# emuell/AFEC

Measured on AMD Instinct MI355X. Metric: audio frames/sec low-level crawl, 44.1kHz 1024-hop, higher is better.
Workload: dtype f64

## Files before the change

### afec_amd/csrc/afx_frames32.hip

```cpp

#include <hip/hip_runtime.h>

#include "afx_internal.h"
#include "afx_device.h"
#include "afx_fft32.h"

namespace afx {
namespace {

using f32x32::cx;

constexpr int kHalfSlots = 1056;
constexpr int kPlane32Bytes = 2 * kHalfSlots * 8;
constexpr int kWaves32 = 8;

template <int POST_ROWS>
struct Lds32 {
  static constexpr int tw = 0;
  static constexpr int post = tw + 32 * 32 * 16;
  static constexpr int dct = post + POST_ROWS * 32 * 16;
  static constexpr int logc = dct + 14 * 16 * 8;
  static constexpr int xchg = logc + 32 * 8;
  static constexpr int total = xchg + kWaves32 * kPlane32Bytes;
};

__device__ __forceinline__ __amdgpu_buffer_rsrc_t table_rsrc(const void* p, int bytes) {
  return __builtin_amdgcn_make_buffer_rsrc(const_cast<void*>(p), 0, bytes, 0x00020000);
}
typedef unsigned int u32x4_t __attribute__((ext_vector_type(4)));
typedef unsigned int u32x2_t __attribute__((ext_vector_type(2)));
__device__ __forceinline__ double2 table_load2(__amdgpu_buffer_rsrc_t rs, int lane_off, int row_off) {
  return __builtin_bit_cast(double2, __builtin_amdgcn_raw_buffer_load_b128(rs, lane_off, row_off, 0));
}
__device__ __forceinline__ double table_load1(__amdgpu_buffer_rsrc_t rs, int lane_off, int row_off) {
  return __builtin_bit_cast(double, __builtin_amdgcn_raw_buffer_load_b64(rs, lane_off, row_off, 0));
}

template <int IMM, bool NT>
__device__ __forceinline__ void dma_piece(const void* gaddr, unsigned lds_base) {
  if constexpr (NT)
    asm volatile("s_mov_b32 m0, %1\n\ts_nop 0\n\tglobal_load_lds_dwordx4 %0, off offset:%2 nt"
                 :: "v"(gaddr), "s"(lds_base), "n"(IMM) : "memory", "m0");
  else
    asm volatile("s_mov_b32 m0, %1\n\ts_nop 0\n\tglobal_load_lds_dwordx4 %0, off offset:%2"
                 :: "v"(gaddr), "s"(lds_base), "n"(IMM) : "memory", "m0");
}
template <bool NT = true>
__device__ __forceinline__ void dma_hop(const float* g, unsigned lds_plane) {
  dma_piece<0, NT>(g, lds_plane);
  dma_piece<512, NT>(g, lds_plane + 512);
  dma_piece<1024, NT>(g, lds_plane + 1024);
  dma_piece<1536, NT>(g, lds_plane + 1536);
  dma_piece<2048, NT>(g, lds_plane + 2048);
  dma_piece<2560, NT>(g, lds_plane + 2560);
  dma_piece<3072, NT>(g, lds_plane + 3072);
  dma_piece<3584, NT>(g, lds_plane + 3584);
}

__device__ __forceinline__ double mag_sqrt_mel(double xr, double xi, double tiny, double three) {
  const double x = fma(xi, xi, fma(xr, xr, tiny));
  const double r = __builtin_amdgcn_rsq(x);
  const double y = x * r;
  return y * fma(-r, y, three);
}

__device__ __forceinline__ void keep_lane0(double& re, double& im, double own_re, double own_im, unsigned long long lane0_mask) {
  unsigned long long saved;
  asm volatile("s_mov_b64 %2, exec\n\ts_mov_b64 exec, %5\n\tv_mov_b64 %0, %3\n\tv_mov_b64 %1, %4\n\ts_mov_b64 exec, %2"
               : "+v"(re), "+v"(im), "=&s"(saved) : "v"(own_re), "v"(own_im), "s"(lane0_mask));
}

__device__ __forceinline__ double half_sum16(double (&a)[16], int lane) {
#pragma unroll
  for (int i = 0; i < 8; ++i) {
    swap16(a[i], a[i + 8]);
    a[i] += a[i + 8];
  }
  const bool b3 = (lane & 8) != 0, b2 = (lane & 4) != 0, b1 = (lane & 2) != 0;
#pragma unroll
  for (int i = 0; i < 4; ++i) {
    const double keep = b3 ? a[i + 4] : a[i];
    const double send = b3 ? a[i] : a[i + 4];
    a[i] = keep + dpp_mov<kDppRor8>(send);
  }
#pragma unroll
  for (int i = 0; i < 2; ++i) {
    const double keep = b2 ? a[i + 2] : a[i];
    const double send = b2 ? a[i] : a[i + 2];
    a[i] = keep + dpp_mov<kDppHalfMirror>(send);
  }
  const double keep = b1 ? a[1] : a[0];
  const double send = b1 ? a[0] : a[1];
  double z = keep + dpp_mov<kDppXor2>(send);
  z += dpp_mov<kDppXor1>(z);
  return z;
}

__device__ const double kLogConst[32] = {1.0 / 23.0, 1.0 / 21.0, 1.0 / 19.0, 1.0 / 17.0, 1.0 / 15.0, 1.0 / 13.0,
                                         1.0 / 11.0, 1.0 / 9.0,  1.0 / 7.0,  1.0 / 5.0,  1.0 / 3.0,  0.693147180559945309417,
                                         0.70710678118654752440, 2e-42,
                                         1e-20, 32.0, 0.38268343236508984, -0.9238795325112867, 1.0 / 738.0,
                                         (double)(85.0f / 100.0), 43.0, -1.0 / 60.0, (double)1e-12f, 3.0,
                                         1.44269504088896340736, 20.0 / 2.30258509299404568402, 2.2250738585072014e-308, 3.33547137486383e-154 , 511.0, 0.0, 0.0, 0.0};
constexpr int kCEps = 14, kC32 = 15, kCRotRe = 16, kCRotIm = 17, kCRoll = 19, kCSqrtMin = 27, kC511 = 28;

__device__ __forceinline__ double log_lds(double x, const double* c) {
  double m = __builtin_amdgcn_frexp_mant(x);
  int e = __builtin_amdgcn_frexp_exp(x);
  const bool lowhalf = m < c[12];
// ... 4 lines not shown
  double p = c[0];
#pragma unroll
  for (int i = 1; i < 11; ++i) p = fma(p, z, c[i]);
  p = fma(p, z, 1.0);
  return fma((double)e, c[11], 2.0 * s * p);
}

__device__ __forceinline__ void finish_mfcc32(double acc, double*& recp, int& left, int stride2, const double* dct,
                                              const double* logc, int lane) {
  const double lg = log_lds(fmax(acc, logc[13]), logc);
  int ln = lane;
  asm volatile("" : "+v"(ln));
  const int n = (ln >> 1) & 15;
  const double2* drow = reinterpret_cast<const double2*>(dct + 16 * (n < kNumCep ? n : 0));
  const int idx = ((ln & 32) + (ln & 1)) << 2;
  const int lo32 = __double2loint(lg), hi32 = __double2hiint(lg);
  double c = 0.0;
#pragma unroll
  for (int m = 0; m < kNumCep; m += 2) {
    const double2 d = drow[m >> 1];
    const double l0 = __hiloint2double(__builtin_amdgcn_ds_bpermute(idx + 8 * m, hi32), __builtin_amdgcn_ds_bpermute(idx + 8 * m, lo32));
    const double l1 = __hiloint2double(__builtin_amdgcn_ds_bpermute(idx + 8 * m + 8, hi32), __builtin_amdgcn_ds_bpermute(idx + 8 * m + 8, lo32));
    c = fma(l0, d.x, c);
    c = fma(l1, d.y, c);
  }
  if (n < kNumCep && left > 0) *recp = c;
  recp += stride2;
  left -= 2;
}

#ifndef AFX_STAMPS
#define AFX_STAMPS 0
#endif
#if AFX_STAMPS
#define AFX_STAMP(i)                                                                           \
  do {                                                                                         \
    unsigned long long t_;                                                                     \
    asm volatile("s_memtime %0\n\ts_waitcnt lgkmcnt(0)" : "=s"(t_));                           \
    stamp_acc[i] += (unsigned)(t_ - stamp_prev);                                               \
    stamp_prev = t_;                                                                           \
  } while (0)
#else
#define AFX_STAMP(i)
#endif


template <int FEAT, bool SCALED>
__global__ __launch_bounds__(kWaves32 * 64) void frames32_kernel(const FrameArgs a) {
  constexpr bool MAGS = (FEAT == 4 || FEAT == 6);
  constexpr bool MAGS_UPPER = (FEAT == 4);
  constexpr int kMelEarly = 4;
  constexpr bool LO_LDS = (FEAT >= 2 && FEAT <= 4) || FEAT == 6;
  constexpr bool kHopNt = !LO_LDS;
  constexpr bool kLoNt = true;
  constexpr bool STATS = (FEAT >= 1 && FEAT <= 3) || FEAT == 5;
  constexpr bool MOMENTS34 = (FEAT != 5);
  constexpr bool PAIRS = STATS;
  constexpr bool STORE = (FEAT == 2 || FEAT == 3);
  constexpr bool UPPER = (FEAT == 3);
  constexpr int MR = (FEAT >= 1) ? 16 : kMel32Rows;
  using Map = Lds32<kMel32Rows>;
  extern __shared__ __align__(16) unsigned char lds_raw[];
  const int lane = threadIdx.x & 63;
  const int wave = __builtin_amdgcn_readfirstlane(threadIdx.x >> 6);
  const int h = lane >> 5, q = lane & 31;

  copy_lds_table(lds_raw + Map::tw, a.tw32, 32 * 32 * 16, threadIdx.x, kWaves32 * 64);
  copy_lds_table(lds_raw + Map::post, a.post32, kMel32Rows * 32 * 16, threadIdx.x, kWaves32 * 64);
  copy_lds_table(lds_raw + Map::dct, a.dct, 14 * 16 * 8, threadIdx.x, kWaves32 * 64);
  copy_lds_table(lds_raw + Map::logc, kLogConst, 32 * 8, threadIdx.x, kWaves32 * 64);
#if AFX_STAMPS
  unsigned stamp_acc[16] = {};
  unsigned long long life_core0, life_real0;
  asm volatile("s_memtime %0\n\ts_memrealtime %1\n\ts_waitcnt lgkmcnt(0)" : "=s"(life_core0), "=s"(life_real0));
  const bool stamping = (wave == 0) && a.stamps != nullptr;
  unsigned long long stamp_prev = 0;
#endif
  __syncthreads();

  const __amdgpu_buffer_rsrc_t win_rs = table_rsrc(a.win32, 32 * 32 * 16);
  const __amdgpu_buffer_rsrc_t mel_rs = table_rsrc(a.melw32, kMel32Pairs * 32 * 8);
  const int q16 = 16 * q, q8 = 8 * q;
  const double2* const tw = reinterpret_cast<const double2*>(lds_raw + Map::tw) + q;
  const double2* const post = reinterpret_cast<const double2*>(lds_raw + Map::post) + q;
  const double* const dct = reinterpret_cast<const double*>(lds_raw + Map::dct);
  const double* const logc = reinterpret_cast<const double*>(lds_raw + Map::logc);
  const int stride2 = 2 * a.lay.stride;
  double* const plane = reinterpret_cast<double*>(lds_raw + Map::xchg + wave * kPlane32Bytes) + kHalfSlots * h;
  double* const pw = plane + q;
  using lds_vdouble = volatile __attribute__((address_space(3))) double;
  lds_vdouble* const pr = (lds_vdouble*)(plane + 33 * q);
  const int partner = (lane & 32) + ((32 - q) & 31);
  const int dh = (lane >> 4) & 1, drow = lane >> 5, dq = 2 * (lane & 15);
  typedef __attribute__((address_space(3))) void lvoid;
  unsigned char* const plane_bytes = lds_raw + Map::xchg + wave * kPlane32Bytes;
  const unsigned plane_lds = __builtin_amdgcn_readfirstlane((unsigned)(size_t)(lvoid*)plane_bytes);
  double k_tiny = 2.2250738585072014e-308, k_three = 3.0;
  unsigned long long k_lane0 = 0x0000000100000001ull;
  asm volatile("" : "+s"(k_tiny), "+s"(k_three), "+s"(k_lane0));
  lds_vdouble* const hop = (lds_vdouble*)(plane_bytes + 256 * h + 8 * q);

  const float* const pcm = reinterpret_cast<const float*>(a.pcm);

  const int n_items = (a.n_chunks + 1) >> 1;
  const int n_static = min((int)(gridDim.x * kWaves32), n_items);
  for (int slot = blockIdx.x * kWaves32 + wave; slot < n_items;) {
    const int ci = 2 * slot + h;
    const bool have = ci < a.n_chunks;
    const Chunk ch = a.chunks[have ? ci : 2 * slot];
    const int nfr = have ? ch.nframes : 0;
    const double sc = ch.scale;
    const int total = max(__builtin_amdgcn_readlane(nfr, 0), __builtin_amdgcn_readlane(nfr, 32));
    const float2* src = reinterpret_cast<const float2*>(pcm + ch.sample_off) + q;
    const int cid = 2 * slot + dh;
    const bool have_d = cid < a.n_chunks;
    const Chunk chd = a.chunks[have_d ? cid : 2 * slot];
    const int last_d = max((have_d ? (int)chd.nframes : 0) - 1, 0);
    const float* const dsrc = pcm + chd.sample_off + 64 * (16 + drow) + 2 * dq;

    double lo[16];
    if constexpr (!LO_LDS) {
      const double* const src8 = reinterpret_cast<const double*>(src);
#pragma unroll
      for (int r = 0; r < 16; ++r) lo[r] = src8[32 * r];
    } else {
      dma_hop<kLoNt>(dsrc - kHop, plane_lds + 8192);
    }
    dma_hop<kHopNt>(dsrc, plane_lds);

    double mel_acc = 0.0;
    double* recp = a.rec + ((int64_t)ch.frame0 + (q & 1)) * a.lay.stride + a.lay.mfcc + ((q >> 1) & 15);
    int left = nfr - (q & 1);

    double2 w[32];
#pragma unroll
    for (int r = 0; r < 32; ++r) w[r] = table_load2(win_rs, q16, 512 * r);

#if AFX_STAMPS
    asm volatile("s_memtime %0\n\ts_waitcnt lgkmcnt(0)" : "=s"(stamp_prev));
#endif
    for (int fi = 0; fi < total; ++fi) {
      cx<double> v[32];
      {
        double nx[16];
        asm volatile("s_waitcnt vmcnt(0)" ::: "memory");
        AFX_STAMP(0);
#pragma unroll
        for (int r = 0; r < 16; ++r) nx[r] = hop[64 * r];
        __builtin_amdgcn_sched_barrier(0);
        if constexpr (LO_LDS) {
          const double* const lo_rows = reinterpret_cast<const double*>(plane_bytes + 8192 + 256 * h) + q;
#pragma unroll
          for (int r = 0; r < 16; ++r) lo[r] = lo_rows[64 * r];
        }
        double hop_sq = 0.0, hop_max = 0.0;
#pragma unroll
        for (int j = 0; j < 8; ++j) {
          auto first = [](double pair) { return __int_as_float(__double2loint(pair)); };
          auto second = [](double pair) { return __int_as_float(__double2hiint(pair)); };
          const double ar = pcm_double<SCALED>(first(lo[j]), sc), ai = pcm_double<SCALED>(second(lo[j]), sc);
          const double br = pcm_double<SCALED>(first(lo[j + 8]), sc), bi = pcm_double<SCALED>(second(lo[j + 8]), sc);
          const double cr = pcm_double<SCALED>(first(nx[j]), sc), ci = pcm_double<SCALED>(second(nx[j]), sc);
          const double dr = pcm_double<SCALED>(first(nx[j + 8]), sc), di = pcm_double<SCALED>(second(nx[j + 8]), sc);
          if constexpr (MAGS) {
            hop_sq = fma(ar, ar, fma(ai, ai, fma(br, br, fma(bi, bi, hop_sq))));
            hop_max = fmax(fmax(hop_max, fmax(fabs(ar), fabs(ai))), fmax(fabs(br), fabs(bi)));
          }
          const double par = ar * w[j].x, pai = ai * w[j].y, pbr = br * w[j + 8].x, pbi = bi * w[j + 8].y;
          const double t0r = fma(cr, w[j + 16].x, par), t0i = fma(ci, w[j + 16].y, pai);
          const double t1r = fma(-cr, w[j + 16].x, par), t1i = fma(-ci, w[j + 16].y, pai);
          const double t2r = fma(dr, w[j + 24].x, pbr), t2i = fma(di, w[j + 24].y, pbi);
          const double t3r = fma(-dr, w[j + 24].x, pbr), t3i = fma(-di, w[j + 24].y, pbi);
          v[j] = {t0r + t2r, t0i + t2i};
          v[j + 16] = {t0r - t2r, t0i - t2i};
          v[j + 8] = {t1r + t3i, t1i - t3r};
          v[j + 24] = {t1r - t3i, t1i + t3r};
        }
        if constexpr (!LO_LDS) {
#pragma unroll
          for (int r = 0; r < 16; ++r) lo[r] = nx[r];
        }
        if constexpr (MAGS) {
          if (a.mask & ((1u << 11) | (1u << 12))) {
            hop_sq += dpp_or_zero<kDppXor1>(hop_sq);      hop_max = fmax(hop_max, dpp_mov<kDppXor1>(hop_max));
            hop_sq += dpp_or_zero<kDppXor2>(hop_sq);      hop_max = fmax(hop_max, dpp_mov<kDppXor2>(hop_max));
            hop_sq += dpp_or_zero<kDppHalfMirror>(hop_sq); hop_max = fmax(hop_max, dpp_mov<kDppHalfMirror>(hop_max));
            hop_sq += dpp_or_zero<kDppMirror>(hop_sq);    hop_max = fmax(hop_max, dpp_mov<kDppMirror>(hop_max));
            const double sq_h = h ? read_lane<32>(hop_sq) + read_lane<48>(hop_sq) : read_lane<0>(hop_sq) + read_lane<16>(hop_sq);
            const double mx_h = h ? fmax(read_lane<32>(hop_max), read_lane<48>(hop_max)) : fmax(read_lane<0>(hop_max), read_lane<16>(hop_max));
            if (q == 0 && fi < nfr) {
              double* const rec = a.rec + ((int64_t)ch.frame0 + fi) * a.lay.stride;
              if ((a.mask & (1u << 11)) && a.lay.amp_peak >= 0) rec[a.lay.amp_peak] = mx_h;
              if ((a.mask & (1u << 12)) && a.lay.amp_rms >= 0) rec[a.lay.amp_rms] = nan_to_zero(sqrt(sq_h / (double)kHop));
            }
          }
        }
      }
      __builtin_amdgcn_sched_barrier(0);
      AFX_STAMP(1);
      f32x32::dft32_rest(v);
      __builtin_amdgcn_sched_barrier(0);
      AFX_STAMP(2);

      double2 t[32];
      auto load_tw = [&](int g) {
#pragma unroll
        for (int j = 2 * g; j < 2 * g + 2; ++j)
#pragma unroll
          for (int i = 0; i < 4; ++i)
            if (j + 8 * i != 0) t[j + 8 * i] = tw[32 * (j + 8 * i)];
      };
      auto bfly_tw = [&](int g) {
#pragma unroll
        for (int j = 2 * g; j < 2 * g + 2; ++j) {
          const cx<double> w1{t[j + 8].x, t[j + 8].y}, w2{t[j + 16].x, t[j + 16].y}, w3{t[j + 24].x, t[j + 24].y};
          if (j == 0) f32x32::radix4_tw3(v[0], v[8], v[16], v[24], w1, w2, w3);
          else f32x32::radix4_tw4(v[j], v[j + 8], v[j + 16], v[j + 24], cx<double>{t[j].x, t[j].y}, w1, w2, w3);
        }
      };
      {
        double re[32], im[32];
#pragma unroll
        for (int k1 = 0; k1 < 32; ++k1) pw[33 * k1] = v[k1].re;
#pragma unroll
        for (int n2 = 0; n2 < 32; ++n2) re[n2] = pr[n2];
#pragma unroll
        for (int k1 = 0; k1 < 32; ++k1) pw[33 * k1] = v[k1].im;
#pragma unroll
        for (int n2 = 0; n2 < 32; ++n2) im[n2] = pr[n2];
        load_tw(0);
        load_tw(1);
#pragma unroll
        for (int n2 = 0; n2 < 32; ++n2) v[n2] = {re[n2], im[n2]};
      }
      asm volatile("s_waitcnt lgkmcnt(0)" ::: "memory");
      AFX_STAMP(3);
      dma_hop<kHopNt>(dsrc + (size_t)min(fi + 1, last_d) * kHop, plane_lds);
      __builtin_amdgcn_sched_barrier(0);

      bfly_tw(0);
      load_tw(2);
      __builtin_amdgcn_sched_barrier(0);
      bfly_tw(1);
      load_tw(3);
      __builtin_amdgcn_sched_barrier(0);
      bfly_tw(2);
      bfly_tw(3);
      __builtin_amdgcn_sched_barrier(0);
      AFX_STAMP(4);
      f32x32::dft32_rest(v);
      __builtin_amdgcn_sched_barrier(0);
      AFX_STAMP(5);

      double mag[MR];
      cx<double> pp[MR];
      double2 pw2[MR];
      double mwt[kMel32Pairs];
      double s1 = 0.0, s2 = 0.0, sj = 0.0, sjj = 0.0, s3 = 0.0, s4 = 0.0, prod_a = 1.0, prod_b = 1.0;
      double jq = 0.0, pa = 0.0;
      double jmir = 0.0;
      double mir[4] = {0.0, 0.0, 0.0, 0.0}, cmid = 0.0;
      double* const park = reinterpret_cast<double*>(plane_bytes + 8192 + 4352 * h);
      auto mag_row = [&]() -> double* {
        int fl = fi, ql = lane;
        asm volatile("" : "+v"(ql), "+s"(fl));
        const int64_t mrow = (fl < nfr) ? (int64_t)ch.frame0 + fl : a.mag_spare_row;
        return a.mag_out + mrow * 1024 + (ql & 31);
      };
      double band26 = 0.0, band27 = 0.0;
      double* rowd = nullptr;
      double* rowm = nullptr;
      auto mag_rows = [&]() {
        rowd = mag_row();
        int ql = lane;
        asm volatile("" : "+v"(ql));
        rowm = rowd + 1024 - 2 * (ql & 31);
      };
      auto store_mag = [&](double* p, double value) { __builtin_nontemporal_store(value > logc[kCSqrtMin] ? value : 0.0, p); };
      if (STATS) {
        int ql = lane;
        asm volatile("" : "+v"(ql));
        jq = (double)((ql & 31) - 1);
        if (PAIRS) jmir = (double)(767 - (ql & 31));
      }
      auto accumulate_at = [&](double value, double j, bool in_range, double* store_at, bool all_in_range) {
        const bool audible = value > logc[kCSqrtMin];
        const bool ok = in_range && audible;
        const double m = ok ? value : 0.0;
        if (STORE && store_at) *store_at = all_in_range ? m : (audible ? value : 0.0);
        const double m2 = m * m;
// ... 263 lines not shown
          pa += dpp_or_zero<kDppRowBcast15, 0xA>(pa);  pb += dpp_or_zero<kDppRowBcast15, 0xA>(pb);
          const int last_idx = base_idx + (22 << 2);
          const double tot_a = __hiloint2double(__builtin_amdgcn_ds_bpermute(last_idx, __double2hiint(pa)),
                                                __builtin_amdgcn_ds_bpermute(last_idx, __double2loint(pa)));
          pb += tot_a;
          const unsigned long long ma = __ballot((hq & 1) == 0 && (hq >> 1) < 12 && pa < pivot);
          const unsigned long long mb = __ballot((hq & 1) == 0 && (hq >> 1) < 13 && pb < pivot);
          const unsigned halfmask_shift = ln & 32;
          const int rstar = __popc((unsigned)(ma >> halfmask_shift)) + __popc((unsigned)(mb >> halfmask_shift));
          const int prev = rstar - 1;
          const int slot = (prev < 12) ? prev : prev - 12;
          const int idx_a = base_idx + ((2 * (slot & 15)) << 2);
          const double base_a = __hiloint2double(__builtin_amdgcn_ds_bpermute(idx_a, __double2hiint(pa)),
                                                 __builtin_amdgcn_ds_bpermute(idx_a, __double2loint(pa)));
          const double base_b = __hiloint2double(__builtin_amdgcn_ds_bpermute(idx_a, __double2hiint(pb)),
                                                 __builtin_amdgcn_ds_bpermute(idx_a, __double2loint(pb)));
          const double before = (rstar == 0) ? 0.0 : ((prev < 12) ? base_a : base_b);
          double xs;
          bool okq;
          int bins_before;
          if constexpr (PAIRS) {
            const bool parked_m = rstar >= 21;
            const int prow = (rstar < 12) ? rstar : (parked_m ? 36 - rstar : 0);
            xs = park[32 * prow + (parked_m ? 31 - hq : hq)];
#pragma unroll
            for (int r = 12; r < 16; ++r) xs = (rstar == r) ? mag[r] : xs;
            xs = (rstar == 16) ? cmid : xs;
            double xm = mir[0];
#pragma unroll
            for (int i = 1; i < 4; ++i) xm = (rstar == 20 - i) ? mir[i] : xm;
            const int ridx = base_idx + ((31 - hq) << 2);
            const double xrev = __hiloint2double(__builtin_amdgcn_ds_bpermute(ridx, __double2hiint(xm)),
                                                 __builtin_amdgcn_ds_bpermute(ridx, __double2loint(xm)));
            xs = (rstar >= 17 && rstar <= 20) ? xrev : xs;
            okq = (rstar == 0) ? (hq != 0) : ((rstar == 16) ? (hq == 0) : ((rstar == 24) ? (hq <= 1) : (rstar < 24)));
            bins_before = (rstar < 16) ? 32 * rstar - (rstar > 0 ? 1 : 0) : ((rstar == 16) ? 511 : 512 + 32 * (rstar - 17));
          }
          xs = okq ? xs : 0.0;
          const double run = halfwave_scan_incl(xs);
          const unsigned long long mrow = __ballot(okq && (before + run) < pivot);
          const int in_row = __popc((unsigned)(mrow >> halfmask_shift));
          const int below = bins_before + in_row;
          int cnt = (pivot > 0.0) ? below + 1 : 0;
          cnt = cnt > kBinCount ? kBinCount : cnt;
          if (live && hq == 0) tmp[7] = (double)cnt;
          __builtin_amdgcn_sched_barrier(0);

#pragma unroll
          for (int r = 0; r < 32; ++r) w[r] = table_load2(win_rs, q16, 512 * r);
          if constexpr (LO_LDS) dma_hop<kLoNt>(dsrc + (size_t)min(fi + 1, last_d) * kHop - kHop, plane_lds + 8192);
        }
        if (fi & 1) finish_mfcc32(mel_acc, recp, left, stride2, dct, logc, lane);
        AFX_STAMP(9);
#if AFX_STAMPS
        stamp_acc[15] += 1;
#endif
      }
    }
    if (total & 1) finish_mfcc32(mel_acc, recp, left, stride2, dct, logc, lane);
    unsigned drawn = 0;
    if (lane == 0) drawn = atomicAdd(a.queue, 1u);
    slot = n_static + (int)((unsigned)__builtin_amdgcn_readfirstlane(drawn) - a.queue_base);
  }
#if AFX_STAMPS
  if (stamping && lane == 0)
    for (int i = 0; i < 16; ++i) atomicAdd(&a.stamps[i], (unsigned long long)stamp_acc[i]);
  if (a.stamps != nullptr && lane == 0) {
    unsigned long long life_core1, life_real1;
    asm volatile("s_memtime %0\n\ts_memrealtime %1\n\ts_waitcnt lgkmcnt(0)" : "=s"(life_core1), "=s"(life_real1));
    unsigned long long* const l = a.stamps + 16 + 4 * ((blockIdx.x & 255) * 8 + wave);
    l[0] = life_core0; l[1] = life_core1; l[2] = life_real0; l[3] = life_real1;
  }
#endif
}

__global__ __launch_bounds__(256) void stats32_finish_kernel(const FrameArgs a, int64_t n_frames) {
  const int64_t f = (int64_t)blockIdx.x * 256 + threadIdx.x;
  if (f >= n_frames) return;
  const double* t = a.stat_tmp + f * kStatTmp;
  const double s1 = t[0], s2 = t[1], sj = t[2], sjj = t[3], s3 = t[4], s4 = t[5], slog = t[6], cnt = t[7];
  double* const rec = a.rec + f * a.lay.stride;
  const double n = (double)kBinCount, inv_n = 1.0 / (double)kBinCount;
  if (a.mask & (1u << 1)) rec[a.lay.srms] = nan_to_zero(sqrt(s2 * inv_n));
  if (a.mask & 0x3Cu) {
    double cen = 0.0, spr = 0.0;
    if (s1 != 0.0) {
      cen = sj / s1;
      spr = (sjj - cen * sj) / s1;
    }
    if (a.lay.centroid >= 0) rec[a.lay.centroid] = cen;
    if (a.lay.spread >= 0) rec[a.lay.spread] = spr;
    if (a.mask & 0x30u) {
      double sk = 0.0, ku = 0.0;
      if (fabs(spr) > (double)1e-12f) {
        const double inv = 1.0 / spr, c2 = cen * cen;
        const double m3 = s3 - 3.0 * cen * s2 + 3.0 * c2 * s1 - n * c2 * cen;
        const double m4 = s4 - 4.0 * cen * s3 + 6.0 * c2 * s2 - 4.0 * c2 * cen * s1 + n * c2 * c2;
        const double i2 = inv * inv;
        sk = m3 * i2 * inv * inv_n;
        ku = m4 * i2 * i2 * inv_n - 3.0;
      }
      if (a.lay.skew >= 0) rec[a.lay.skew] = sk;
      if (a.lay.kurt >= 0) rec[a.lay.kurt] = ku;
    }
  }
  if (a.mask & (1u << 7)) {
    const double gm = fast_exp(slog * inv_n);
    const double am = s1 * inv_n;
    const double fl = (am == 0.0) ? 0.0 : gm / am;
    const double d = lin_to_db(fl) * (-1.0 / 60.0);
    rec[a.lay.flatness] = nan_to_zero(d < 1.0 ? d : 1.0);
  }
  if (a.mask & (1u << 6)) rec[a.lay.rolloff] = cnt * (double)(kSampleRate / (kFft / 2));
}

// ... 62 lines not shown
```

### afec_amd/csrc/afx_batch_plan.cpp

```cpp

#include <algorithm>
#include <cmath>
#include <cstdlib>
#include <cstring>
#include <new>

#include "afx_host.h"

namespace afx {
namespace host {

#define AFX_FIELD(name, lay, width, bit) {&afx_out::name, &afx_stats_out::name, &afx::RecordLayout::lay, width, bit}
const FieldDesc kFields[AFX_NUM_SERIES] = {
    AFX_FIELD(mfcc, mfcc, 14, AFX_D_MFCC),
    AFX_FIELD(spectral_rms, srms, 1, AFX_D_SPECTRAL_RMS),
    AFX_FIELD(spectral_centroid, centroid, 1, AFX_D_SPECTRAL_CENTROID),
    AFX_FIELD(spectral_spread, spread, 1, AFX_D_SPECTRAL_SPREAD),
    AFX_FIELD(spectral_skewness, skew, 1, AFX_D_SPECTRAL_SKEWNESS),
    AFX_FIELD(spectral_kurtosis, kurt, 1, AFX_D_SPECTRAL_KURTOSIS),
    AFX_FIELD(spectral_rolloff, rolloff, 1, AFX_D_SPECTRAL_ROLLOFF),
    AFX_FIELD(spectral_flatness, flatness, 1, AFX_D_SPECTRAL_FLATNESS),
    AFX_FIELD(spectral_flux, flux, 1, AFX_D_SPECTRAL_FLUX),
    AFX_FIELD(spectrum_bands, bands, 28, AFX_D_SPECTRUM_BANDS),
    AFX_FIELD(amplitude_peak, amp_peak, 1, AFX_D_AMPLITUDE_PEAK),
// ... 109 lines not shown
  const afx_plan* plan = p.plan;
  b->halfwave = plan->halfwave && frames_use_halfwave(p.fmask, plan->desc.precision, p.src.dtype) &&
                (plan->halfwave == 2 || p.frames >= 8 * (int64_t)plan->cu_count * frames32_waves_per_block() * 2);
  if (b->halfwave && frames32_class(p.fmask) >= 2) b->mag_wanted = true;
  p.waves_per_block = b->halfwave ? frames32_waves_per_block() : frames_waves_per_block(p.fmask);
  p.slots = (int64_t)plan->cu_count * p.waves_per_block * (b->halfwave ? 2 : 1);
}

int choose_chunk_frames(const Planner& p) {
  const afx_batch* b = p.b;
  constexpr double kHalfwavePrologue = 0.5;
  int K = 32;
  double best = 1e300;
  const int k_step = (p.mask & AFX_D_AUTO_CORRELATION) ? 2 : 1;
  for (int k = k_step; k <= 32; k += k_step) {
    int64_t nchunks = 0;
    for (int i = 0; i < p.src.n_bufs; ++i) nchunks += (b->frame_offset[i + 1] - b->frame_offset[i] + k - 1) / k;
    const double prologue = b->halfwave ? kHalfwavePrologue : 0.5;
    constexpr double kTailWeight = 0.4;
    const double cost = b->halfwave ? ((double)p.frames + (double)nchunks * prologue) / (double)p.slots + kTailWeight * k
                                    : (double)((nchunks + p.slots - 1) / p.slots) * (k + prologue);
    if (cost < best - 1e-9 || (std::fabs(cost - best) <= 1e-9 && k > K)) { best = cost; K = k; }
  }
  return K;
}

void cut_chunks(Planner& p, int K) {
  afx_batch* b = p.b;
  const afx_plan* plan = p.plan;
  std::vector<Chunk>& chunks = b->h_chunks;
  std::vector<ChunkRemaining>& remaining = b->h_remaining;
  b->chunk_frames = K;
  const bool guided = b->halfwave && K >= 8 && !(p.mask & (kTimeBits | kWhitenBits | AFX_D_BAND_FEATURES | AFX_D_SPECTRAL_FLUX));
  const int Ks = guided ? K / 4 : K;
  for (int i = 0; i < p.src.n_bufs; ++i) {
    const int64_t f = b->frame_offset[i + 1] - b->frame_offset[i];
    const int64_t f_long = guided ? (f * 7 / 8) / K * K : f;
    for (int64_t f0 = 0; f0 < f;) {
      const int k = (f0 < f_long) ? K : Ks;
      remaining.push_back((ChunkRemaining)std::min<int64_t>(p.length(i) - f0 * plan->desc.hop_size, 1 << 30));
      Chunk c;
      c.sample_off = b->arena_off[i] + f0 * plan->desc.hop_size;
      c.frame0 = (int32_t)(b->frame_offset[i] + f0);
      c.nframes = (int16_t)std::min<int64_t>(k, f - f0);
      c.flags = (int16_t)(f0 == 0 ? kChunkFirstOfBuffer : 0);
      c.scale = p.scale_of(i);
      chunks.push_back(c);
      f0 += k;
    }
  }
  if (guided)
    std::stable_sort(chunks.begin(), chunks.end(), [](const Chunk& x, const Chunk& y) { return x.nframes > y.nframes; });
  b->n_chunks = (int)chunks.size();
  const int64_t wave_items = b->halfwave ? (b->n_chunks + 1) / 2 : b->n_chunks;
  b->grid_blocks = (int)std::min<int64_t>((wave_items + p.waves_per_block - 1) / p.waves_per_block, (int64_t)plan->cu_count);
  if (b->grid_blocks < 1) b->grid_blocks = 1;
}

void cut_whitening_chunks(Planner& p) {
  afx_batch* b = p.b;
  const int n_bufs = p.src.n_bufs, K = b->chunk_frames;
  constexpr int64_t kWholeFileFrames = 128;
  const bool whole_files = n_bufs >= 768;
  std::vector<Chunk>& wchunks = b->h_wchunks;
  std::vector<int32_t>& chunk_first = b->h_chunk_first;
  chunk_first.assign((size_t)n_bufs + 1, 0);
  for (int i = 0; i < n_bufs; ++i) {
    const int64_t f = b->frame_offset[i + 1] - b->frame_offset[i];
    chunk_first[(size_t)i] = (int32_t)wchunks.size();
    const int64_t step = (whole_files && f <= kWholeFileFrames) ? std::max<int64_t>(f, 1) : K;
    if (f > step) b->need_follow = true;
    for (int64_t f0 = 0; f0 < f; f0 += step) {
      Chunk c;
      c.sample_off = b->arena_off[i] + f0 * p.plan->desc.hop_size;
      c.frame0 = (int32_t)(b->frame_offset[i] + f0);
      c.nframes = (int16_t)std::min<int64_t>(step, f - f0);
      c.flags = (int16_t)(f0 == 0 ? kChunkFirstOfBuffer : 0);
      c.scale = p.scale_of(i);
      wchunks.push_back(c);
    }
  }
  chunk_first[(size_t)n_bufs] = (int32_t)wchunks.size();
  b->n_wchunks = (int)wchunks.size();
}

struct Reserver {
  afx_plan* plan;
  Workspace* ws;
  hipStream_t stream;
  hipError_t e = hipSuccess;
  const char* what = "";
  struct Table { void** dst; size_t off, bytes; };
  std::vector<Table> tables;
  std::vector<unsigned char> image;
  template <typename T>
  bool table(T** dst, const void* src, size_t bytes, const char* name) {
    what = name;
    *dst = nullptr;
    if (!bytes) return true;
    const size_t off = (image.size() + 63) & ~(size_t)63;
    image.resize(off + bytes);
    std::memcpy(image.data() + off, src, bytes);
    tables.push_back(Table{(void**)dst, off, bytes});
    return true;
  }
  template <typename T>
  bool operator()(Workspace::Buf& buf, T** dst, size_t bytes, const char* name) {
    what = name;
    if ((e = ws_reserve(plan, buf, bytes)) != hipSuccess) return false;
// ... 198 lines not shown
```

### afec_amd/csrc/afx_batch_run.cpp

```cpp

#include <algorithm>
#include <cmath>
#include <cstdio>

#include "afx_host.h"

namespace afx {
namespace host {

#if defined(AFX_STAMPS) && AFX_STAMPS
unsigned long long* g_stamp_buf = nullptr;
#endif

namespace {

void stats_regimes(const std::vector<int64_t>& offset, afx::StatsArgs* sa) {
  sa->small_rows = 0;
  sa->need_long = 0;
  for (size_t i = 0; i + 1 < offset.size(); ++i) {
    const int64_t n = offset[i + 1] - offset[i];
    if (n >= 2 && n <= 128) sa->small_rows = std::max<int32_t>(sa->small_rows, (int32_t)n);
    else sa->need_long = 1;
  }
}
// ... 74 lines not shown
  const int frame_class = b->halfwave ? frames32_class(frames_mask(b->mask)) : -1;
  const uint32_t post_amplitude = (b->total_frames > 0 && (frame_class == 2 || frame_class == 3))
                                      ? (b->mask & (AFX_D_AMPLITUDE_PEAK | AFX_D_AMPLITUDE_RMS)) : 0u;
  if (!(b->total_frames > 0 && ((b->mask & kTimeBits) || post_amplitude))) return AFX_OK;
  const bool time_side = b->plan->side_stream && frames_mask(b->mask) != 0 && !(b->mask & AFX_D_RHYTHM);
  hipStream_t ts = b->stream;
  if (time_side) {
    HIP_TRY(hipEventRecord(b->ws->ev_fork, b->stream));
    HIP_TRY(hipStreamWaitEvent(b->ws->side_stream, b->ws->ev_fork, 0));
    ts = b->ws->side_stream;
  }
  TimeArgs ta{};
  ta.pcm = b->d_pcm; ta.chunks = b->d_chunks; ta.remaining = b->d_rem; ta.n_chunks = b->n_chunks;
  ta.pcm_dtype = b->pcm_dtype; ta.rec = b->d_rec; ta.lay = b->lay;
  ta.t1 = t.t1_f64; ta.t2 = t.t2_f64; ta.post = t.post_f64;
  ta.amplitude = post_amplitude;
  const bool want_hop = (b->mask & (AFX_D_AMPLITUDE_SILENCE | AFX_D_AMPLITUDE_ENVELOPE)) || post_amplitude;
  ta.hop_here = (want_hop && (b->mask & AFX_D_F0)) ? 1u : 0u;
  if (want_hop && !ta.hop_here) HIP_TRY(launch_hop(ta, ts));
  if (b->mask & AFX_D_F0) {
    ta.queue = b->ws->queues.take(kQueuePitch, b->n_chunks);
    HIP_TRY(launch_pitch(ta, ts));
  }
  if (b->mask & AFX_D_AUTO_CORRELATION) {
    ta.queue = b->ws->queues.take(kQueueAcorr, b->n_chunks);
    HIP_TRY(launch_acorr(ta, ts));
  }
  if (time_side) HIP_TRY(hipEventRecord(b->ws->ev_time_join, ts));
  *on_side = time_side;
  return AFX_OK;
}

int launch_frame_kernel(afx_batch* b) {
  if (!frames_mask(b->mask)) return AFX_OK;
  const DeviceTables& t = b->plan->dev;
  FrameArgs a{};
  a.pcm = b->d_pcm;
  a.chunks = b->d_chunks;
  a.n_chunks = b->n_chunks;
  a.mask = frames_mask(b->mask);
  a.rec = b->d_rec;
  a.lay = b->lay;
  a.mag_out = b->d_mag;
  a.win = t.win; a.t1 = t.t1; a.t2 = t.t2; a.post = t.post; a.melw = t.melw; a.dct = t.dct;
  a.win32 = t.win32; a.tw32 = t.tw32; a.post32 = t.post32; a.melw32 = t.melw32;
#if defined(AFX_STAMPS) && AFX_STAMPS
  if (!g_stamp_buf) { HIP_TRY(hipMalloc((void**)&g_stamp_buf, (16 + 8192) * 8)); HIP_TRY(hipMemset(g_stamp_buf, 0, (16 + 8192) * 8)); }
  a.stamps = g_stamp_buf;
#endif
  if (!b->halfwave) {
    HIP_TRY(launch_frames(a, b->plan->desc.precision, b->pcm_dtype, b->grid_blocks, b->stream));
    return AFX_OK;
  }
  const WorkQueue q = b->ws->queues.take(kQueueFrames32, (b->n_chunks + 1) / 2);
  a.queue = q.counter;
  a.queue_base = q.base;
  a.stat_tmp = b->d_stat_tmp;
  a.mag_spare_row = b->total_frames;
  HIP_TRY(launch_frames32(a, b->grid_blocks, b->stream, b->total_frames, b->pcm_dtype == kPcmScaledF32));
  return AFX_OK;
}

int launch_band_kernel(afx_batch* b) {
  const bool bands28_later = b->halfwave && (b->mask & AFX_D_SPECTRUM_BANDS);
  const bool stats_later = b->halfwave && frames32_class(frames_mask(b->mask)) == 4;
  if (!((b->mask & (AFX_D_BAND_FEATURES | AFX_D_SPECTRAL_FLUX)) || bands28_later)) return AFX_OK;
  BandArgs ba{};
  ba.mag = b->d_mag; ba.chunks = b->d_chunks; ba.n_chunks = b->n_chunks; ba.rec = b->d_rec; ba.lay = b->lay;
  ba.flags = ((b->mask & AFX_D_BAND_FEATURES) ? kBandsFeatures : 0) | ((b->mask & AFX_D_SPECTRAL_FLUX) ? kBandsFlux : 0) |
             (bands28_later ? kBandsSpectrum : 0) | (stats_later ? kBandsStats : 0);
  ba.stat_tmp = b->d_stat_tmp;
  ba.queue = b->ws->queues.take(kQueueBands, b->n_chunks);
  HIP_TRY(launch_bands(ba, b->stream));
  if (stats_later) {
    FrameArgs fa{};
    fa.mask = frames_mask(b->mask); fa.rec = b->d_rec; fa.lay = b->lay; fa.stat_tmp = b->d_stat_tmp;
    HIP_TRY(launch_stats32_finish(fa, b->stream, b->total_frames));
  }
  return AFX_OK;
}

int launch_whitening(afx_batch* b) {
  if (!(b->mask & kWhitenBits)) return AFX_OK;
  WhitenArgs wa{};
  wa.mag = b->d_mag; wa.frame_offset = b->d_frame_offset; wa.n_bufs = b->n_bufs; wa.mask = b->mask;
  wa.chunk_first = b->d_chunk_first; wa.chunks = b->d_wchunks; wa.n_chunks = b->n_wchunks;
  wa.chunk_frames = b->chunk_frames; wa.follower = b->d_follower; wa.need_follow = b->need_follow ? 1 : 0;
  wa.rec = b->d_rec; wa.lay = b->lay;
  wa.decay = std::pow(0.001, (double)((float)b->plan->desc.hop_size / (float)b->plan->desc.sample_rate) / 22.0);
  wa.floor_value = 1.e-4;
  wa.queue = b->ws->queues.take(kQueueWhiten, b->n_wchunks);
  HIP_TRY(launch_whiten(wa, b->stream));
  return AFX_OK;
}

int batch_run_enqueue(afx_batch* b) {
  b->ran = true;
  bool time_side = false;
  int st = launch_time_domain(b, &time_side);
  if (st != AFX_OK) return st;
  if ((st = rhythm_fork(b, time_side)) != AFX_OK) return st;
  if (b->d_efflen) {
    const double k = std::log(10.0) / 20.0;
    HIP_TRY(launch_effective_length(b->d_pcm, b->pcm_dtype, b->d_spans, b->n_bufs, std::exp(-48.0 * k), std::exp(-24.0 * k),
                                    std::exp(-12.0 * k), b->d_efflen, b->stream));
  }
  if (b->total_frames == 0) {
    if ((st = launch_statistics(b)) != AFX_OK) return st;
    return rhythm_join(b);
  }
  if ((st = launch_frame_kernel(b)) != AFX_OK) return st;
  if ((st = launch_band_kernel(b)) != AFX_OK) return st;
  if (time_side) HIP_TRY(hipStreamWaitEvent(b->stream, b->ws->ev_time_join, 0));
  if ((st = launch_whitening(b)) != AFX_OK) return st;
  if ((st = launch_statistics(b)) != AFX_OK) return st;
  return rhythm_join(b);
}

}

#if defined(AFX_STAMPS) && AFX_STAMPS
void stamps_report() {
  if (!g_stamp_buf) return;
  unsigned long long h[16];
  if (hipMemcpy(h, g_stamp_buf, sizeof h, hipMemcpyDeviceToHost) == hipSuccess && h[15]) {
    static const char* names[10] = {"wait DMA+window", "hop+convert", "P1", "exchange", "DMA issue+twiddle", "P2",
                                    "untangle", "mel rows", "win issue+reduce", "log+DCT"};
    unsigned long long tot = 0;
    for (int i = 0; i < 10; ++i) tot += h[i];
    std::fprintf(stderr, "[afx stamps] %llu stamped iterations (2 frames each), %.0f cycles per iteration\n", h[15], (double)tot / h[15]);
    for (int i = 0; i < 10; ++i) std::fprintf(stderr, "[afx stamps] %-18s %8.0f cycles  %5.1f %%\n", names[i], (double)h[i] / h[15], 100.0 * h[i] / tot);
    static unsigned long long life[8192];
    if (hipMemcpy(life, g_stamp_buf + 16, sizeof life, hipMemcpyDeviceToHost) == hipSuccess) {
      unsigned long long r0 = ~0ull, r1 = 0;
      double sum_core = 0, sum_real = 0;
      double wsum[8] = {}, wmin[8], wmax[8] = {}, wend[8] = {};
      int wn[8] = {};
      for (int w = 0; w < 8; ++w) wmin[w] = 1e30;
      for (int i = 0; i < 2048; ++i) {
        if (!life[4 * i + 1]) continue;
        r0 = std::min(r0, life[4 * i + 2]); r1 = std::max(r1, life[4 * i + 3]);
      }
      for (int i = 0; i < 2048; ++i) {
        if (!life[4 * i + 1]) continue;
        const int w = i & 7;
        const double dr = (double)(life[4 * i + 3] - life[4 * i + 2]) / 100.0;
        sum_core += (double)(life[4 * i + 1] - life[4 * i]); sum_real += dr * 100.0;
        wsum[w] += dr; wmin[w] = std::min(wmin[w], dr); wmax[w] = std::max(wmax[w], dr); ++wn[w];
        wend[w] += (double)(life[4 * i + 3] - r0) / 100.0;
      }
      std::fprintf(stderr, "[afx stamps] last launch: span first-entry..last-exit %.1f us, core clock %.3f GHz\n", (double)(r1 - r0) / 100.0, sum_core / sum_real * 0.1);
      for (int w = 0; w < 8; ++w)
        if (wn[w]) std::fprintf(stderr, "[afx stamps]   wave %d: life mean %.1f us (min %.1f, max %.1f), mean exit at %.1f us\n", w, wsum[w] / wn[w], wmin[w], wmax[w], wend[w] / wn[w]);
    }
    hipMemset(g_stamp_buf, 0, (16 + 8192) * 8);
  }
}
#endif

}
}

using namespace afx::host;

extern "C" {

int afx_batch_run(afx_batch* b) {
  if (!b) return fail(AFX_ERR_INVALID_ARG, "null batch");
  HIP_TRY(hipSetDevice(b->plan->desc.device));
  Workspace* const ws = b->ws;
  if (ws && ws->queues.needs_repair()) HIP_TRY(ws->queues.repair(b->stream, ws->side_stream));
  const int st = batch_run_enqueue(b);
  if (st != AFX_OK && ws) ws->queues.mark_failed();
  return st;
}

int afx_batch_sync(afx_batch* b) {
  if (!b) return fail(AFX_ERR_INVALID_ARG, "null batch");
  HIP_TRY(hipStreamSynchronize(b->stream));
  return AFX_OK;
}

int afx_batch_run_timed(afx_batch* b, int32_t steps, float* elapsed_ms) {
  if (!b || steps < 1 || !elapsed_ms) return fail(AFX_ERR_INVALID_ARG, "bad argument");
// ... 14 lines not shown
```

### afec_amd/csrc/afx_internal.h

```cpp
#pragma once

#include <hip/hip_runtime.h>
#include <stdint.h>

namespace afx {
constexpr uint32_t kFramesWholeSpectrum = 1u << 31;
constexpr uint32_t kFramesStatsLater = 1u << 30;
constexpr int kStatTmp = 10;

constexpr int kSampleRate = 44100;
constexpr int kFft = 2048;
constexpr int kHop = 1024;
constexpr int kHalf = kFft / 2;
constexpr int kNumCep = 14;
constexpr int kNumBands = 28;
constexpr int kNumSub = 14;
constexpr int kFirstBin = 1;
constexpr int kLastBin = 738;
constexpr int kBinCount = 738;

constexpr int kMelLo[kNumCep] = {1, 1, 5, 10, 17, 25, 35, 48, 64, 83, 108, 139, 177, 225};
constexpr int kMelHi[kNumCep] = {3, 8, 15, 23, 33, 46, 62, 81, 106, 137, 175, 223, 283, 358};
constexpr int kMelRows = 6;

constexpr bool mel_touches(int f, int r) { return kMelLo[f] <= 64 * r + 63 && kMelHi[f] >= 64 * r; }
constexpr int mel_pair_count() {
  int n = 0;
  for (int r = 0; r < kMelRows; ++r)
    for (int f = 0; f < kNumCep; ++f) n += mel_touches(f, r) ? 1 : 0;
  return n;
}
constexpr int kMelPairs = mel_pair_count();
constexpr int mel_pair_index(int r, int f) {
  int n = 0;
  for (int rr = 0; rr < kMelRows; ++rr)
    for (int ff = 0; ff < kNumCep; ++ff) {
      if (rr == r && ff == f) return n;
      n += mel_touches(ff, rr) ? 1 : 0;
    }
  return -1;
}

constexpr int kMel32Rows = 12;
constexpr bool mel32_touches(int f, int r) { return kMelLo[f] <= 32 * r + 31 && kMelHi[f] >= 32 * r; }
constexpr int mel32_pair_count() {
  int n = 0;
  for (int r = 0; r < kMel32Rows; ++r)
    for (int f = 0; f < kNumCep; ++f) n += mel32_touches(f, r) ? 1 : 0;
  return n;
}
constexpr int kMel32Pairs = mel32_pair_count();
constexpr int mel32_pair_index(int r, int f) {
  int n = 0;
  for (int rr = 0; rr < kMel32Rows; ++rr)
    for (int ff = 0; ff < kNumCep; ++ff) {
      if (rr == r && ff == f) return n;
// ... 248 lines not shown
```

Before: 496.9 million.

## Load next hop directly into registers for FEAT 0 with cache-line touch prefetch

After: 471.4 million. -5.1%, worse.

```diff
diff --git a/afec_amd/csrc/afx_frames32.hip b/afec_amd/csrc/afx_frames32.hip
--- a/afec_amd/csrc/afx_frames32.hip
+++ b/afec_amd/csrc/afx_frames32.hip
@@ -55,6 +55,20 @@
   dma_piece<2560, NT>(g, lds_plane + 2560);
   dma_piece<3072, NT>(g, lds_plane + 3072);
   dma_piece<3584, NT>(g, lds_plane + 3584);
+}
+
+#ifndef AFX_HOP_TOUCH_POLICY
+#define AFX_HOP_TOUCH_POLICY 2
+#endif
+__device__ __forceinline__ int touch_line(const float* p) {
+  const int* const ip = reinterpret_cast<const int*>(p);
+#if AFX_HOP_TOUCH_POLICY == 0
+  return *reinterpret_cast<const volatile int*>(ip);
+#elif AFX_HOP_TOUCH_POLICY == 1
+  return __builtin_nontemporal_load(ip);
+#else
+  return __hip_atomic_load(ip, __ATOMIC_RELAXED, __HIP_MEMORY_SCOPE_AGENT);
+#endif
 }
 
 __device__ __forceinline__ double mag_sqrt_mel(double xr, double xi, double tiny, double three) {
@@ -165,6 +179,7 @@
   constexpr int kMelEarly = 4;
   constexpr bool LO_LDS = (FEAT >= 2 && FEAT <= 4) || FEAT == 6;
   constexpr bool kHopNt = !LO_LDS;
+  constexpr bool HOP_REGS = (FEAT == 0);
   constexpr bool kLoNt = true;
   constexpr bool STATS = (FEAT >= 1 && FEAT <= 3) || FEAT == 5;
   constexpr bool MOMENTS34 = (FEAT != 5);
@@ -232,14 +247,27 @@
     const float* const dsrc = pcm + chd.sample_off + 64 * (16 + drow) + 2 * dq;
 
     double lo[16];
+    const double* const src8 = reinterpret_cast<const double*>(src);
     if constexpr (!LO_LDS) {
-      const double* const src8 = reinterpret_cast<const double*>(src);
 #pragma unroll
       for (int r = 0; r < 16; ++r) lo[r] = src8[32 * r];
     } else {
       dma_hop<kLoNt>(dsrc - kHop, plane_lds + 8192);
     }
-    dma_hop<kHopNt>(dsrc, plane_lds);
+    double nx[16];
+    const int last = max(nfr - 1, 0);
+    auto hop_line = [&](int f) {
+      int ql = lane;
+      asm volatile("" : "+v"(ql));
+      return reinterpret_cast<const float*>(src8 + 512 * (size_t)(1 + min(f, last))) + 30 * (ql & 31);
+    };
+    int touched = 0;
+    if constexpr (HOP_REGS) {
+#pragma unroll
+      for (int r = 0; r < 16; ++r) nx[r] = __builtin_nontemporal_load(src8 + 32 * (16 + r));
+    } else {
+      dma_hop<kHopNt>(dsrc, plane_lds);
+    }
 
     double mel_acc = 0.0;
     double* recp = a.rec + ((int64_t)ch.frame0 + (q & 1)) * a.lay.stride + a.lay.mfcc + ((q >> 1) & 15);
@@ -255,11 +283,14 @@
     for (int fi = 0; fi < total; ++fi) {
       cx<double> v[32];
       {
-        double nx[16];
         asm volatile("s_waitcnt vmcnt(0)" ::: "memory");
         AFX_STAMP(0);
-#pragma unroll
-        for (int r = 0; r < 16; ++r) nx[r] = hop[64 * r];
+        if constexpr (HOP_REGS) {
+          asm volatile("" :: "v"(touched));
+        } else {
+#pragma unroll
+          for (int r = 0; r < 16; ++r) nx[r] = hop[64 * r];
+        }
         __builtin_amdgcn_sched_barrier(0);
         if constexpr (LO_LDS) {
           const double* const lo_rows = reinterpret_cast<const double*>(plane_bytes + 8192 + 256 * h) + q;
@@ -289,7 +320,10 @@
           v[j + 8] = {t1r + t3i, t1i - t3r};
           v[j + 24] = {t1r - t3i, t1i + t3r};
         }
-        if constexpr (!LO_LDS) {
+        if constexpr (HOP_REGS) {
+#pragma unroll
+          for (int r = 0; r < 16; ++r) asm volatile("v_mov_b64 %0, %1" : "=v"(lo[r]) : "v"(nx[r]));
+        } else if constexpr (!LO_LDS) {
 #pragma unroll
           for (int r = 0; r < 16; ++r) lo[r] = nx[r];
         }
@@ -346,9 +380,14 @@
 #pragma unroll
         for (int n2 = 0; n2 < 32; ++n2) v[n2] = {re[n2], im[n2]};
       }
-      asm volatile("s_waitcnt lgkmcnt(0)" ::: "memory");
-      AFX_STAMP(3);
-      dma_hop<kHopNt>(dsrc + (size_t)min(fi + 1, last_d) * kHop, plane_lds);
+      if constexpr (HOP_REGS) {
+        AFX_STAMP(3);
+        touched = touch_line(hop_line(fi + 2));
+      } else {
+        asm volatile("s_waitcnt lgkmcnt(0)" ::: "memory");
+        AFX_STAMP(3);
+        dma_hop<kHopNt>(dsrc + (size_t)min(fi + 1, last_d) * kHop, plane_lds);
+      }
       __builtin_amdgcn_sched_barrier(0);
 
       bfly_tw(0);
@@ -718,6 +757,11 @@
         }
         if (fi & 1) finish_mfcc32(mel_acc, recp, left, stride2, dct, logc, lane);
         AFX_STAMP(9);
+        if constexpr (HOP_REGS) {
+          const double* const nsrc = src8 + 512 * (size_t)(1 + min(fi + 1, last));
+#pragma unroll
+          for (int r = 0; r < 16; ++r) nx[r] = __builtin_nontemporal_load(nsrc + 32 * r);
+        }
 #if AFX_STAMPS
         stamp_acc[15] += 1;
 #endif
```

## Schedule frames32 work per workgroup group instead of per wave

Applied to the files above, without the earlier changes.

Result: slower. 509.1 million before, 470.7 million after (-7.5%).

```diff
diff --git a/afec_amd/csrc/afx_batch_plan.cpp b/afec_amd/csrc/afx_batch_plan.cpp
--- a/afec_amd/csrc/afx_batch_plan.cpp
+++ b/afec_amd/csrc/afx_batch_plan.cpp
@@ -185,9 +185,12 @@
   if (guided)
     std::stable_sort(chunks.begin(), chunks.end(), [](const Chunk& x, const Chunk& y) { return x.nframes > y.nframes; });
   b->n_chunks = (int)chunks.size();
-  const int64_t wave_items = b->halfwave ? (b->n_chunks + 1) / 2 : b->n_chunks;
-  b->grid_blocks = (int)std::min<int64_t>((wave_items + p.waves_per_block - 1) / p.waves_per_block, (int64_t)plan->cu_count);
-  if (b->grid_blocks < 1) b->grid_blocks = 1;
+  if (b->halfwave) {
+    b->grid_blocks = frames32_grid_blocks(b->n_chunks, plan->cu_count);
+  } else {
+    b->grid_blocks = (int)std::min<int64_t>(((int64_t)b->n_chunks + p.waves_per_block - 1) / p.waves_per_block, (int64_t)plan->cu_count);
+    if (b->grid_blocks < 1) b->grid_blocks = 1;
+  }
 }
 
 void cut_whitening_chunks(Planner& p) {
diff --git a/afec_amd/csrc/afx_batch_run.cpp b/afec_amd/csrc/afx_batch_run.cpp
--- a/afec_amd/csrc/afx_batch_run.cpp
+++ b/afec_amd/csrc/afx_batch_run.cpp
@@ -150,7 +150,7 @@
     HIP_TRY(launch_frames(a, b->plan->desc.precision, b->pcm_dtype, b->grid_blocks, b->stream));
     return AFX_OK;
   }
-  const WorkQueue q = b->ws->queues.take(kQueueFrames32, (b->n_chunks + 1) / 2);
+  const WorkQueue q = b->ws->queues.take(kQueueFrames32, frames32_queue_items(b->n_chunks));
   a.queue = q.counter;
   a.queue_base = q.base;
   a.stat_tmp = b->d_stat_tmp;
@@ -222,12 +222,13 @@
   if (!g_stamp_buf) return;
   unsigned long long h[16];
   if (hipMemcpy(h, g_stamp_buf, sizeof h, hipMemcpyDeviceToHost) == hipSuccess && h[15]) {
-    static const char* names[10] = {"wait DMA+window", "hop+convert", "P1", "exchange", "DMA issue+twiddle", "P2",
-                                    "untangle", "mel rows", "win issue+reduce", "log+DCT"};
+    constexpr int kStages = 12;
+    static const char* names[kStages] = {"wait DMA+window", "hop+convert", "P1", "exchange", "DMA issue+twiddle", "P2",
+                                         "untangle", "mel rows", "win issue+reduce", "log+DCT", "barrier S1|S2", "barrier S2|S1"};
     unsigned long long tot = 0;
-    for (int i = 0; i < 10; ++i) tot += h[i];
+    for (int i = 0; i < kStages; ++i) tot += h[i];
     std::fprintf(stderr, "[afx stamps] %llu stamped iterations (2 frames each), %.0f cycles per iteration\n", h[15], (double)tot / h[15]);
-    for (int i = 0; i < 10; ++i) std::fprintf(stderr, "[afx stamps] %-18s %8.0f cycles  %5.1f %%\n", names[i], (double)h[i] / h[15], 100.0 * h[i] / tot);
+    for (int i = 0; i < kStages; ++i) std::fprintf(stderr, "[afx stamps] %-18s %8.0f cycles  %5.1f %%\n", names[i], (double)h[i] / h[15], 100.0 * h[i] / tot);
     static unsigned long long life[8192];
     if (hipMemcpy(life, g_stamp_buf + 16, sizeof life, hipMemcpyDeviceToHost) == hipSuccess) {
       unsigned long long r0 = ~0ull, r1 = 0;
diff --git a/afec_amd/csrc/afx_frames32.hip b/afec_amd/csrc/afx_frames32.hip
--- a/afec_amd/csrc/afx_frames32.hip
+++ b/afec_amd/csrc/afx_frames32.hip
@@ -4,6 +4,7 @@
 #include "afx_internal.h"
 #include "afx_device.h"
 #include "afx_fft32.h"
+#include "afx_groups32.h"
 
 namespace afx {
 namespace {
@@ -21,8 +22,22 @@
   static constexpr int dct = post + POST_ROWS * 32 * 16;
   static constexpr int logc = dct + 14 * 16 * 8;
   static constexpr int xchg = logc + 32 * 8;
-  static constexpr int total = xchg + kWaves32 * kPlane32Bytes;
+  static constexpr int draw = xchg + kWaves32 * kPlane32Bytes;
+  static constexpr int total = draw + 16;
 };
+static_assert(kWaves32 == kGroupWaves32, "a group is one chunk pair per wave of the workgroup");
+
+#ifndef AFX_LOCKSTEP0
+#define AFX_LOCKSTEP0 0
+#endif
+constexpr int lockstep_of_class(int feat) { return feat == 0 ? AFX_LOCKSTEP0 : 0; }
+
+__device__ __forceinline__ void phase_barrier() {
+  __builtin_amdgcn_sched_barrier(0);
+  __builtin_amdgcn_s_barrier();
+  __builtin_amdgcn_sched_barrier(0);
+}
+
 
 __device__ __forceinline__ __amdgpu_buffer_rsrc_t table_rsrc(const void* p, int bytes) {
   return __builtin_amdgcn_make_buffer_rsrc(const_cast<void*>(p), 0, bytes, 0x00020000);
@@ -215,19 +230,36 @@
 
   const float* const pcm = reinterpret_cast<const float*>(a.pcm);
 
-  const int n_items = (a.n_chunks + 1) >> 1;
-  const int n_static = min((int)(gridDim.x * kWaves32), n_items);
-  for (int slot = blockIdx.x * kWaves32 + wave; slot < n_items;) {
+  const int n_groups = frames32_group_count(a.n_chunks);
+  const int n_static = frames32_static_groups(n_groups, (int)gridDim.x);
+  volatile __attribute__((address_space(3))) unsigned* const drawn_lds =
+      (volatile __attribute__((address_space(3))) unsigned*)(lds_raw + Map::draw);
+  typedef const __attribute__((address_space(4))) int32_t cint;
+  cint* const chunk_words = (cint*)(uintptr_t)a.chunks;
+  static_assert(sizeof(Chunk) == 24 && offsetof(Chunk, nframes) == 12, "frames of chunk c: low half of word 6 c + 3");
+  constexpr int LOCK = lockstep_of_class(FEAT);
+  const bool late = wave >= kWaves32 / 2;
+  if (LOCK >= 2 && late) __builtin_amdgcn_s_setprio(1);
+  unsigned draw_parity = 0;
+  for (int group = blockIdx.x; group < n_groups;) {
+    const int slot = group * kWaves32 + wave;
     const int ci = 2 * slot + h;
     const bool have = ci < a.n_chunks;
-    const Chunk ch = a.chunks[have ? ci : 2 * slot];
+    const Chunk ch = a.chunks[have ? ci : frames32_group_first(group)];
     const int nfr = have ? ch.nframes : 0;
+    int total = 0;
+#pragma unroll
+    for (int c = 0; c < kGroupChunks32; ++c) {
+      const int cg = frames32_group_first(group) + c;
+      const int nf = (int)(int16_t)chunk_words[6 * (cg < a.n_chunks ? cg : frames32_group_first(group)) + 3];
+      total = max(total, cg < a.n_chunks ? nf : 0);
+    }
+    total = __builtin_amdgcn_readfirstlane(total);
     const double sc = ch.scale;
-    const int total = max(__builtin_amdgcn_readlane(nfr, 0), __builtin_amdgcn_readlane(nfr, 32));
     const float2* src = reinterpret_cast<const float2*>(pcm + ch.sample_off) + q;
     const int cid = 2 * slot + dh;
     const bool have_d = cid < a.n_chunks;
-    const Chunk chd = a.chunks[have_d ? cid : 2 * slot];
+    const Chunk chd = a.chunks[have_d ? cid : frames32_group_first(group)];
     const int last_d = max((have_d ? (int)chd.nframes : 0) - 1, 0);
     const float* const dsrc = pcm + chd.sample_off + 64 * (16 + drow) + 2 * dq;
 
@@ -252,6 +284,7 @@
 #if AFX_STAMPS
     asm volatile("s_memtime %0\n\ts_waitcnt lgkmcnt(0)" : "=s"(stamp_prev));
 #endif
+    if (LOCK && late) phase_barrier();
     for (int fi = 0; fi < total; ++fi) {
       cx<double> v[32];
       {
@@ -345,6 +378,10 @@
         load_tw(1);
 #pragma unroll
         for (int n2 = 0; n2 < 32; ++n2) v[n2] = {re[n2], im[n2]};
+      }
+      if (LOCK) {
+        phase_barrier();
+        AFX_STAMP(10);
       }
       asm volatile("s_waitcnt lgkmcnt(0)" ::: "memory");
       AFX_STAMP(3);
@@ -718,15 +755,21 @@
         }
         if (fi & 1) finish_mfcc32(mel_acc, recp, left, stride2, dct, logc, lane);
         AFX_STAMP(9);
+        if (LOCK) {
+          phase_barrier();
+          AFX_STAMP(11);
+        }
 #if AFX_STAMPS
         stamp_acc[15] += 1;
 #endif
       }
     }
+    if (LOCK && !late) phase_barrier();
     if (total & 1) finish_mfcc32(mel_acc, recp, left, stride2, dct, logc, lane);
-    unsigned drawn = 0;
-    if (lane == 0) drawn = atomicAdd(a.queue, 1u);
-    slot = n_static + (int)((unsigned)__builtin_amdgcn_readfirstlane(drawn) - a.queue_base);
+    if (wave == 0 && lane == 0) drawn_lds[draw_parity] = atomicAdd(a.queue, (unsigned)frames32_group_pairs(group, a.n_chunks));
+    __syncthreads();
+    group = frames32_drawn_group((unsigned)__builtin_amdgcn_readfirstlane(drawn_lds[draw_parity]) - a.queue_base, n_static);
+    draw_parity ^= 1u;
   }
 #if AFX_STAMPS
   if (stamping && lane == 0)
diff --git a/afec_amd/csrc/afx_groups32.h b/afec_amd/csrc/afx_groups32.h
--- /dev/null
+++ b/afec_amd/csrc/afx_groups32.h
@@ -0,0 +1,45 @@
+#pragma once
+
+#include <cstdint>
+
+namespace afx {
+
+constexpr int kGroupWaves32 = 8;
+constexpr int kGroupChunks32 = 2 * kGroupWaves32;
+
+constexpr int frames32_queue_items(int n_chunks) { return n_chunks > 0 ? (n_chunks + 1) / 2 : 0; }
+constexpr int frames32_group_count(int n_chunks) { return n_chunks > 0 ? (n_chunks + kGroupChunks32 - 1) / kGroupChunks32 : 0; }
+constexpr int frames32_grid_blocks(int n_chunks, int cu_count) {
+  const int g = frames32_group_count(n_chunks);
+  return g < 1 ? 1 : (g < cu_count ? g : cu_count);
+}
+constexpr int frames32_static_groups(int n_groups, int grid_blocks) { return n_groups < grid_blocks ? n_groups : grid_blocks; }
+constexpr int frames32_group_pairs(int g, int n_chunks) {
+  return frames32_queue_items(n_chunks) - g * kGroupWaves32 < kGroupWaves32 ? frames32_queue_items(n_chunks) - g * kGroupWaves32 : kGroupWaves32;
+}
+constexpr int frames32_drawn_group(unsigned drawn, int n_static) { return n_static + (int)((drawn + kGroupWaves32 - 1) / kGroupWaves32); }
+constexpr int frames32_group_first(int g) { return g * kGroupChunks32; }
+constexpr int frames32_group_end(int g, int n_chunks) { return (g + 1) * kGroupChunks32 < n_chunks ? (g + 1) * kGroupChunks32 : n_chunks; }
+
+template <typename FramesOfChunk>
+int frames32_group_trip(FramesOfChunk nframes, int n_chunks, int g) {
+  int trip = 0;
+  for (int c = frames32_group_first(g); c < frames32_group_end(g, n_chunks); ++c) trip = nframes(c) > trip ? nframes(c) : trip;
+  return trip;
+}
+
+struct Groups32Cost {
+  int n_groups;
+  int64_t frames;
+  int64_t slots;
+  int64_t padded() const { return slots - frames; }
+};
+template <typename FramesOfChunk>
+Groups32Cost frames32_groups_cost(FramesOfChunk nframes, int n_chunks) {
+  Groups32Cost c{frames32_group_count(n_chunks), 0, 0};
+  for (int i = 0; i < n_chunks; ++i) c.frames += nframes(i);
+  for (int g = 0; g < c.n_groups; ++g) c.slots += (int64_t)kGroupChunks32 * frames32_group_trip(nframes, n_chunks, g);
+  return c;
+}
+
+}
diff --git a/afec_amd/csrc/afx_internal.h b/afec_amd/csrc/afx_internal.h
--- a/afec_amd/csrc/afx_internal.h
+++ b/afec_amd/csrc/afx_internal.h
@@ -2,6 +2,8 @@
 
 #include <hip/hip_runtime.h>
 #include <stdint.h>
+
+#include "afx_groups32.h"
 
 namespace afx {
 constexpr uint32_t kFramesWholeSpectrum = 1u << 31;
```
